# xyfJASON/ctrlora

Measured on NVIDIA H100. Metric: ddim_steps_per_sec, higher is better.
Workload: dtype fp16 (fp32 accumulate)

## Files before the change

ctrlora_b200/csrc/gemm_sm90.cu:

```cuda
#include "gemm_sm90.cuh"
#include "wgmma.cuh"
#include "ctrlora_b200.h"
#include <stdio.h>
#include <string.h>

namespace ctrl {

__device__ __forceinline__ uint32_t pack_h2(float a, float b) {
    __half2 h = __floats2half2_rn(a, b);
    return *reinterpret_cast<uint32_t*>(&h);
}

template <int CW>
__device__ __forceinline__ void epilogue_chunk(const GemmKParams& p, float* v, int c, int bn_out, int n0, bool row_ok,
                                               long long m, int img, int tok) {
    const int nbase = n0 + c;
    const bool full_chunk = (c + CW <= bn_out) && (nbase + CW <= p.N);
    if (!row_ok) return;
    if (p.rowbias) {
        const float* rb = p.rowbias + static_cast<long long>(img) * p.rowbias_ld + nbase;
        if (full_chunk && (p.rowbias_ld & 3) == 0) {
#pragma unroll
            for (int q = 0; q < CW / 4; ++q) {
                const float4 b4 = __ldg(reinterpret_cast<const float4*>(rb) + q);
                v[4 * q] += b4.x; v[4 * q + 1] += b4.y; v[4 * q + 2] += b4.z; v[4 * q + 3] += b4.w;
            }
        } else {
#pragma unroll
            for (int j = 0; j < CW; ++j)
                if (nbase + j < p.N) v[j] += __ldg(rb + j);
        }
    }
    if (p.out_scale != 1.0f) {
#pragma unroll
        for (int j = 0; j < CW; ++j) v[j] *= p.out_scale;
    }
    if (p.residual && p.residual_f32) {
        const float* rp = reinterpret_cast<const float*>(p.residual) + m * p.ldr + nbase;
        if (full_chunk && (p.ldr & 3) == 0) {
#pragma unroll
            for (int q = 0; q < CW / 4; ++q) {
                const float4 r4 = __ldg(reinterpret_cast<const float4*>(rp) + q);
                v[4 * q] += r4.x; v[4 * q + 1] += r4.y; v[4 * q + 2] += r4.z; v[4 * q + 3] += r4.w;
            }
        } else {
#pragma unroll
            for (int j = 0; j < CW; ++j)
                if (c + j < bn_out && nbase + j < p.N) v[j] += rp[j];
        }
    } else if (p.residual) {
        const __half* rp = p.residual + m * p.ldr + nbase;
        if (full_chunk && (p.ldr & 7) == 0) {
            uint4 u[CW / 8];
#pragma unroll
            for (int q = 0; q < CW / 8; ++q) u[q] = __ldg(reinterpret_cast<const uint4*>(rp) + q);
#pragma unroll
            for (int q = 0; q < CW / 8; ++q) {
                const __half2* h = reinterpret_cast<const __half2*>(&u[q]);
#pragma unroll
                for (int e = 0; e < 4; ++e) {
                    const float2 f = __half22float2(h[e]);
                    v[q * 8 + e * 2] += f.x;
                    v[q * 8 + e * 2 + 1] += f.y;
                }
            }
        } else {
#pragma unroll
            for (int j = 0; j < CW; ++j)
                if (c + j < bn_out && nbase + j < p.N) v[j] += __half2float(rp[j]);
        }
    }
    int seg = 0, nloc = nbase;
    if (p.seg_width > 0) { seg = nbase / p.seg_width; nloc = nbase - seg * p.seg_width; }
    if (p.transposed[seg]) {
        __half* o = reinterpret_cast<__half*>(p.out[seg]) + (static_cast<long long>(img) * p.seg_width + nloc) * p.tok_pad + tok;
#pragma unroll
        for (int j = 0; j < CW; ++j)
            if (c + j < bn_out && nbase + j < p.N) o[static_cast<long long>(j) * p.tok_pad] = __float2half_rn(v[j]);
        if (p.dup_out) {
            __half* o2 = p.dup_out + m * p.dup_ld + nloc;
#pragma unroll
            for (int j = 0; j < CW; ++j)
                if (c + j < bn_out && nbase + j < p.N) o2[j] = __float2half_rn(v[j]);
        }
    } else if (p.out_f32) {
        float* o = reinterpret_cast<float*>(p.out[seg]) + m * p.ldc + nloc;
        if (full_chunk && (p.ldc & 3) == 0) {
#pragma unroll
            for (int q = 0; q < CW / 4; ++q)
                reinterpret_cast<float4*>(o)[q] = make_float4(v[q * 4], v[q * 4 + 1], v[q * 4 + 2], v[q * 4 + 3]);
        } else {
#pragma unroll
            for (int j = 0; j < CW; ++j)
                if (c + j < bn_out && nbase + j < p.N) o[j] = v[j];
        }
    } else {
        __half* o = reinterpret_cast<__half*>(p.out[seg]) + m * p.ldc + nloc;
        if (full_chunk && (p.ldc & 7) == 0) {
#pragma unroll
            for (int q = 0; q < CW / 8; ++q) {
                uint4 u;
                u.x = pack_h2(v[q * 8 + 0], v[q * 8 + 1]);
                u.y = pack_h2(v[q * 8 + 2], v[q * 8 + 3]);
                u.z = pack_h2(v[q * 8 + 4], v[q * 8 + 5]);
                u.w = pack_h2(v[q * 8 + 6], v[q * 8 + 7]);
                reinterpret_cast<uint4*>(o)[q] = u;
            }
        } else {
#pragma unroll
            for (int j = 0; j < CW; ++j)
                if (c + j < bn_out && nbase + j < p.N) o[j] = __float2half_rn(v[j]);
        }
    }
}

struct GemmUnit {
    int mt, nt, it0, it1, ks, slot;
};
__device__ __forceinline__ GemmUnit gemm_unit(const GemmKParams& p, int u, int m_tiles, int k_iters) {
    GemmUnit w;
    int tile;
    if (u < p.tiles_whole) {
        tile = u;
        w.ks = 0; w.slot = -1; w.it0 = 0; w.it1 = k_iters;
    } else {
        const int v = u - p.tiles_whole;
        w.slot = v / p.splits;
        w.ks = v - w.slot * p.splits;
        tile = p.tiles_whole + w.slot;
        w.it0 = w.ks * p.kiters_per_split;
        w.it1 = min(k_iters, w.it0 + p.kiters_per_split);
    }
    w.mt = tile % m_tiles;
    w.nt = tile / m_tiles;
    return w;
}

__device__ __forceinline__ uint32_t epi_addr(uint32_t base, int r, int col) {
    return base + static_cast<uint32_t>(r * (GEMM_EPI_COLS * 4) + ((((col >> 2) ^ (r & 7)) << 4) | ((col & 3) << 2)));
}

template <bool GEGLU, int BN>
__global__ void __launch_bounds__(GEMM_THREADS, 1)
gemm_wgmma_kernel(const __grid_constant__ CUtensorMap tmA, const __grid_constant__ CUtensorMap tmB,
                  const __grid_constant__ CUtensorMap tmA2, const __grid_constant__ CUtensorMap tmB2,
                  const __grid_constant__ GemmKParams p) {
    constexpr int BN_OUT = GEGLU ? BN / 2 : BN;
    constexpr int NACC = BN / 2;
    constexpr int BOX = GEGLU || BN > 256 ? BN / 2 : BN;
    extern __shared__ uint8_t smem_raw[];
    uint8_t* smem = reinterpret_cast<uint8_t*>((reinterpret_cast<uintptr_t>(smem_raw) + 1023) & ~uintptr_t(1023));
    uint64_t* bars = reinterpret_cast<uint64_t*>(smem + GEMM_SMEM_DATA + GEMM_EPI_BYTES);
    uint64_t* full = bars;
    uint64_t* empty = bars + GEMM_MAX_STAGES;
    volatile int* last_flag = reinterpret_cast<volatile int*>(bars + 2 * GEMM_MAX_STAGES);

    pdl_launch_dependents();
    const int warp = uniform_warp_idx();
    const int lane = threadIdx.x & 31;
    const int nstages = p.stages;
    if (threadIdx.x == 0) {
        tma_prefetch_desc(&tmA);
        tma_prefetch_desc(&tmB);
        if (p.kchunks2 > 0) {
            tma_prefetch_desc(&tmA2);
            tma_prefetch_desc(&tmB2);
        }
        for (int i = 0; i < nstages; ++i) {
            mbar_init(&full[i], 1);
            mbar_init(&empty[i], GEMM_CONSUMERS);
        }
        fence_barrier_init();
    }
    __syncthreads();
    pdl_wait();

    const int m_tiles = p.tiles_w * p.tiles_h * p.tiles_b;
    const int main_iters = p.taps * p.kchunks;
    const int k_iters = main_iters + p.kchunks2;

    if (warp < 4) {
        setmaxnreg_dec<GEMM_PRODUCER_REGS>();
        if (warp == 0 && elect_one()) {
            const uint32_t tx_bytes = GEMM_A_BYTES + BN * 128;
            int s = 0;
            uint32_t phase = 0;
            for (int u = blockIdx.x; u < p.units; u += gridDim.x) {
                const GemmUnit w = gemm_unit(p, u, m_tiles, k_iters);
                const int tw = w.mt % p.tiles_w, th = (w.mt / p.tiles_w) % p.tiles_h, tb = w.mt / (p.tiles_w * p.tiles_h);
                const int w0 = tw * p.bw - p.pad, h0 = th * p.bh - p.pad, b0 = tb * p.nb, n0 = w.nt * BN_OUT;
                for (int it = w.it0; it < w.it1; ++it) {
                    mbar_wait_nocall(&empty[s], phase ^ 1);
                    uint8_t* dst = smem + s * p.stage_bytes;
                    mbar_expect_tx(&full[s], tx_bytes);
                    if (it < main_iters) {
                        const int tap = it / p.kchunks, kc = it - tap * p.kchunks, ky = tap / p.kw, kx = tap - ky * p.kw;
                        tma_load_4d(dst, &tmA, &full[s], kc * GEMM_BK, w0 + kx, h0 + ky, b0);
                        tma_load_3d(dst + GEMM_A_BYTES, &tmB, &full[s], kc * GEMM_BK, tap, n0);
                        if (BOX < BN)
                            tma_load_3d(dst + GEMM_A_BYTES + BOX * 128, &tmB, &full[s], kc * GEMM_BK, tap, GEGLU ? p.N + n0 : n0 + BOX);
                    } else {
                        const int c0 = (it - main_iters) * GEMM_BK;
                        tma_load_4d(dst, &tmA2, &full[s], c0, w0 + p.pad, h0 + p.pad, b0);
                        tma_load_3d(dst + GEMM_A_BYTES, &tmB2, &full[s], c0, 0, n0);
                        if (BOX < BN) tma_load_3d(dst + GEMM_A_BYTES + BOX * 128, &tmB2, &full[s], c0, 0, n0 + BOX);
                    }
                    if (++s == nstages) { s = 0; phase ^= 1; }
                }
            }
        }
        return;
    }

    setmaxnreg_inc<GEMM_CONSUMER_REGS>();
    const int ct = threadIdx.x - 128;
    const int wg = ct >> 7, t = ct & 127;
    const uint32_t smem0 = smem_u32(smem);
    const uint32_t stg = smem0 + GEMM_SMEM_DATA + wg * (64 * GEMM_EPI_COLS * 4);
    const int fr = ((t >> 5) << 4) + (lane >> 2), cq = 2 * (lane & 3);
    const int er = t & 63, eh = t >> 6;
    const long long slice = static_cast<long long>(GEMM_BM) * BN;
    int s = 0;
    uint32_t phase = 0;
    for (int u = blockIdx.x; u < p.units; u += gridDim.x) {
        const GemmUnit w = gemm_unit(p, u, m_tiles, k_iters);
        float acc[NACC];
#pragma unroll
        for (int i = 0; i < NACC; ++i) acc[i] = 0.f;
        int prev = -1;
        for (int it = w.it0; it < w.it1; ++it) {
            mbar_wait_nocall(&full[s], phase);
            const uint32_t a_base = smem0 + s * p.stage_bytes + wg * 64 * 128;
            const uint32_t b_base = smem0 + s * p.stage_bytes + GEMM_A_BYTES;
            wgmma_fence();
#pragma unroll
            for (int k = 0; k < GEMM_BK / 16; ++k) {
                const uint32_t sc = (it > w.it0 || k > 0) ? 1u : 0u;
                if constexpr (BN > 256) {
                    WgmmaSS<BN / 2, 0, 0>::mma(acc, wgmma_desc_kmajor(a_base + 32 * k), wgmma_desc_kmajor(b_base + 32 * k), sc);
                    WgmmaSS<BN / 2, 0, 0>::mma(acc + NACC / 2, wgmma_desc_kmajor(a_base + 32 * k),
                                               wgmma_desc_kmajor(b_base + (BN / 2) * 128 + 32 * k), sc);
                } else {
                    WgmmaSS<BN, 0, 0>::mma(acc, wgmma_desc_kmajor(a_base + 32 * k), wgmma_desc_kmajor(b_base + 32 * k), sc);
                }
            }
            wgmma_commit();
            wgmma_wait<1>();
            if (prev >= 0) mbar_arrive(&empty[prev]);
            prev = s;
            if (++s == nstages) { s = 0; phase ^= 1; }
        }
        wgmma_wait<0>();
        wgmma_fence_regs<NACC>(acc);
        mbar_arrive(&empty[prev]);

        if (w.slot >= 0) {
            float* frag0 = p.ws + static_cast<long long>(w.slot) * p.splits * slice + ct * 4;
#pragma unroll
            for (int i = 0; i < NACC / 4; ++i)
                __stcg(reinterpret_cast<float4*>(frag0 + w.ks * slice + i * (GEMM_CONSUMERS * 4)),
                       make_float4(acc[4 * i], acc[4 * i + 1], acc[4 * i + 2], acc[4 * i + 3]));
            __threadfence();
            named_bar_sync(1, GEMM_CONSUMERS);
            if (ct == 0) {
                const unsigned int old = atomicAdd(&p.counters[w.slot], 1u);
                const int last = (old == static_cast<unsigned int>(p.splits - 1));
                if (last) p.counters[w.slot] = 0;
                *last_flag = last;
            }
            named_bar_sync(1, GEMM_CONSUMERS);
            if (!*last_flag) continue;
            __threadfence();
#pragma unroll
            for (int i = 0; i < NACC / 4; ++i) {
                float4 t4 = make_float4(0.f, 0.f, 0.f, 0.f);
                for (int sl = 0; sl < p.splits; ++sl) {
                    const float4 x4 = __ldcg(reinterpret_cast<const float4*>(frag0 + sl * slice + i * (GEMM_CONSUMERS * 4)));
                    t4.x += x4.x; t4.y += x4.y; t4.z += x4.z; t4.w += x4.w;
                }
                acc[4 * i] = t4.x; acc[4 * i + 1] = t4.y; acc[4 * i + 2] = t4.z; acc[4 * i + 3] = t4.w;
            }
        }

        const int n0 = w.nt * BN_OUT;
        auto bias_geglu = [&](int i) {
#pragma unroll
            for (int e = 0; e < 2; ++e) {
                const int n = n0 + 8 * i + cq + e;
                float bv = 0.f, bg = 0.f;
                if (p.bias && n < p.N) {
                    bv = __ldg(p.bias + n);
                    if (GEGLU) bg = __ldg(p.bias + p.N + n);
                }
                acc[4 * i + e] += bv;
                acc[4 * i + 2 + e] += bv;
                if (GEGLU) {
                    acc[4 * i + e] *= gelu_erf_f(acc[4 * (i + BN_OUT / 8) + e] + bg);
                    acc[4 * i + 2 + e] *= gelu_erf_f(acc[4 * (i + BN_OUT / 8) + 2 + e] + bg);
                }
            }
        };
        if (GEGLU) {
#pragma unroll
            for (int i = 0; i < BN_OUT / 8; ++i) bias_geglu(i);
        }
        const int tw = w.mt % p.tiles_w, th = (w.mt / p.tiles_w) % p.tiles_h, tb = w.mt / (p.tiles_w * p.tiles_h);
        const int r = wg * 64 + er;
        const int iw = r % p.bw, ih = (r / p.bw) % p.bh, ib = r / (p.bw * p.bh);
        const int gw = tw * p.bw + iw, gh = th * p.bh + ih, gb = tb * p.nb + ib;
        const bool row_ok = gw < p.W && gh < p.H && gb < p.Bn;
        const long long m = (static_cast<long long>(gb) * p.H + gh) * p.W + gw;
        const int img = row_ok ? static_cast<int>(m / p.rows_per_img) : 0;
        const int tok = row_ok ? static_cast<int>(m % p.rows_per_img) : 0;
        constexpr int NSLAB = (BN_OUT + GEMM_EPI_COLS - 1) / GEMM_EPI_COLS;
#pragma unroll
        for (int sl = 0; sl < NSLAB; ++sl) {
            const int s0 = sl * GEMM_EPI_COLS;
#pragma unroll
            for (int j = 0; j < GEMM_EPI_COLS / 8; ++j) {
                const int i = sl * (GEMM_EPI_COLS / 8) + j;
                if (i >= BN_OUT / 8) break;
                if (!GEGLU) bias_geglu(i);
                const int col = 8 * j + cq;
                asm volatile("st.shared.v2.f32 [%0], {%1, %2};" ::"r"(epi_addr(stg, fr, col)), "f"(acc[4 * i]), "f"(acc[4 * i + 1])
                             : "memory");
                asm volatile("st.shared.v2.f32 [%0], {%1, %2};" ::"r"(epi_addr(stg, fr + 8, col)), "f"(acc[4 * i + 2]),
                             "f"(acc[4 * i + 3])
                             : "memory");
            }
            named_bar_sync(2 + wg, 128);
            constexpr int CW = BN_OUT > 128 ? 16 : 32;
#pragma unroll
            for (int c1 = 0; c1 < 32; c1 += CW) {
                const int c = s0 + 32 * eh + c1;
                if (c < BN_OUT) {
                    float v[CW];
#pragma unroll
                    for (int q = 0; q < CW / 4; ++q) {
                        const float4 x = lds128f(epi_addr(stg, er, 32 * eh + c1 + 4 * q));
                        v[4 * q] = x.x; v[4 * q + 1] = x.y; v[4 * q + 2] = x.z; v[4 * q + 3] = x.w;
                    }
                    epilogue_chunk<CW>(p, v, c, BN_OUT, n0, row_ok, m, img, tok);
                }
            }
            named_bar_sync(2 + wg, 128);
        }
    }
}

typedef CUresult (*PFN_tmapEncodeTiled)(CUtensorMap*, CUtensorMapDataType, cuuint32_t, void*, const cuuint64_t*,
                                        const cuuint64_t*, const cuuint32_t*, const cuuint32_t*, CUtensorMapInterleave,
                                        CUtensorMapSwizzle, CUtensorMapL2promotion, CUtensorMapFloatOOBfill);

PFN_tmapEncodeTiled get_tmap_encoder() {
    static PFN_tmapEncodeTiled fn = nullptr;
    if (!fn) {
        void* ptr = nullptr;
        cudaDriverEntryPointQueryResult q;
        if (cudaGetDriverEntryPoint("cuTensorMapEncodeTiled", &ptr, cudaEnableDefault, &q) != cudaSuccess ||
            q != cudaDriverEntryPointSuccess)
            return nullptr;
        fn = reinterpret_cast<PFN_tmapEncodeTiled>(ptr);
    }
    return fn;
}

static int make_tmap_f16_sw(CUtensorMap* map, const void* base, int rank, const uint64_t* dims, const uint64_t* strides_bytes,
                            const uint32_t* box, CUtensorMapSwizzle swz);
int make_tmap_f16(CUtensorMap* map, const void* base, int rank, const uint64_t* dims, const uint64_t* strides_bytes,
                  const uint32_t* box) {
    return make_tmap_f16_sw(map, base, rank, dims, strides_bytes, box, CU_TENSOR_MAP_SWIZZLE_128B);
}
static int make_tmap_f16_sw(CUtensorMap* map, const void* base, int rank, const uint64_t* dims, const uint64_t* strides_bytes,
                            const uint32_t* box, CUtensorMapSwizzle swz) {
    PFN_tmapEncodeTiled enc = get_tmap_encoder();
    if (!enc) return CTRLORA_ERR_TMAP;
    cuuint64_t gdim[5], gstr[4];
    cuuint32_t bx[5], es[5];
    for (int i = 0; i < rank; ++i) { gdim[i] = dims[i]; bx[i] = box[i]; es[i] = 1; }
    for (int i = 0; i + 1 < rank; ++i) gstr[i] = strides_bytes[i];
    CUresult r = enc(map, CU_TENSOR_MAP_DATA_TYPE_FLOAT16, rank, const_cast<void*>(base), gdim, gstr, bx, es,
                     CU_TENSOR_MAP_INTERLEAVE_NONE, swz, CU_TENSOR_MAP_L2_PROMOTION_L2_256B,
                     CU_TENSOR_MAP_FLOAT_OOB_FILL_NONE);
    if (r != CUDA_SUCCESS) {
        fprintf(stderr, "ctrlora: cuTensorMapEncodeTiled failed (%d) rank %d dims", (int)r, rank);
        for (int i = 0; i < rank; ++i) fprintf(stderr, " %llu", (unsigned long long)dims[i]);
        fprintf(stderr, " box");
        for (int i = 0; i < rank; ++i) fprintf(stderr, " %u", box[i]);
        fprintf(stderr, "\n");
        return CTRLORA_ERR_TMAP;
    }
    return CTRLORA_OK;
}

static int pow2_floor(int x) {
    int p = 1;
    while (p * 2 <= x) p *= 2;
    return p;
}

static int g_num_sms = 0;
static int g_sm_limit = 0;

int persistent_sms() {
    if (g_num_sms == 0) {
        int dev = 0;
        cudaGetDevice(&dev);
        cudaDeviceGetAttribute(&g_num_sms, cudaDevAttrMultiProcessorCount, dev);
        if (g_num_sms <= 0) return 0;
    }
    return g_sm_limit > 0 && g_sm_limit < g_num_sms ? g_sm_limit : g_num_sms;
}

constexpr double GEMM_L2_BPC = 40.0;
constexpr double GEMM_EPI_FIXED = 600.0;
constexpr double GEMM_EPI_PER_COL = 12.0;
constexpr double GEMM_SPLIT_PER_COL = 12.0;
constexpr int GEMM_MAX_AUTO_SPLIT = 8;
static constexpr int GEMM_WIDE_MIN_KITERS = 40;
static bool g_attr_set = false;

template <bool GEGLU, int BN>
static cudaError_t launch_gemm(dim3 grid, cudaStream_t stream, const CUtensorMap& tmA, const CUtensorMap& tmB,
                               const CUtensorMap& tmA2, const CUtensorMap& tmB2, const GemmKParams& p) {
    return launch_pdl(gemm_wgmma_kernel<GEGLU, BN>, grid, dim3(GEMM_THREADS), (size_t)GEMM_SMEM_BYTES, stream, tmA, tmB, tmA2,
                      tmB2, p);
}
template <bool GEGLU, int BN>
static bool set_smem_attr() {
    return cudaFuncSetAttribute(gemm_wgmma_kernel<GEGLU, BN>, cudaFuncAttributeMaxDynamicSharedMemorySize, GEMM_SMEM_BYTES) ==
           cudaSuccess;
}

}

using namespace ctrl;

extern "C" int ctrlora_gemm_f16(const ctrlora_gemm_args* a, void* stream_) {
    cudaStream_t stream = reinterpret_cast<cudaStream_t>(stream_);
    if (!a || !a->a || !a->w || !a->out[0]) return CTRLORA_ERR_ARG;
    if (a->a_c % 8 != 0 || a->a_ld % 8 != 0) return CTRLORA_ERR_ARG;
    if (a->kh != a->kw || (a->kh != 1 && a->kh != 3)) return CTRLORA_ERR_UNSUPPORTED;
    if (a->bf16) return CTRLORA_ERR_UNSUPPORTED;
    GemmKParams p;
    memset(&p, 0, sizeof(p));
    p.W = a->a_w; p.H = a->a_h; p.Bn = a->a_b;
    p.bw = pow2_floor(p.W < 128 ? p.W : 128);
    p.bh = pow2_floor(p.H < 128 / p.bw ? p.H : 128 / p.bw);
    p.nb = 128 / (p.bw * p.bh);
    p.tiles_w = (p.W + p.bw - 1) / p.bw;
    p.tiles_h = (p.H + p.bh - 1) / p.bh;
    p.tiles_b = (p.Bn + p.nb - 1) / p.nb;
    p.N = a->n;
    p.taps = a->kh * a->kw; p.kw = a->kw; p.pad = a->pad;
    p.kchunks = (a->a_c + GEMM_BK - 1) / GEMM_BK;
    p.kchunks2 = a->a2 ? (a->a2_c + GEMM_BK - 1) / GEMM_BK : 0;
    p.geglu = a->geglu;
    const int sms = persistent_sms();
    if (sms <= 0) return CTRLORA_ERR_CUDA;
    const int m_tiles = p.tiles_w * p.tiles_h * p.tiles_b;
    const int k_iters = p.taps * p.kchunks + p.kchunks2;
    const bool explicit_split = a->split_k > 0;
    auto plan = [&](int cand, int S, int* s_eff, int* whole) -> double {
        const int bnt = p.geglu ? 2 * cand : cand;
        const long long tiles = (long long)m_tiles * ((p.N + cand - 1) / cand);
        const int kps = (k_iters + S - 1) / S;
        *s_eff = (k_iters + kps - 1) / kps;
        long long w = *s_eff == 1 ? tiles : explicit_split ? 0 : (tiles / sms) * sms;
        const long long tail = tiles - w;
        if (*s_eff > 1 && (!a->splitk_ws || !a->splitk_counters || tail == 0 ||
                           tail * *s_eff * GEMM_BM * bnt * 4 > a->splitk_ws_bytes || tail > a->splitk_counters_len))
            return -1.0;
        *whole = (int)w;
        const double step = fmax(4.0 * bnt, (double)(GEMM_A_BYTES + bnt * 128) / GEMM_L2_BPC);
        const double epi = GEMM_EPI_FIXED + GEMM_EPI_PER_COL * cand;
        const double t_whole = k_iters * step + epi;
        const double t_split = kps * step + epi + GEMM_SPLIT_PER_COL * bnt * (1 + *s_eff);
        return (double)((w + sms - 1) / sms) * t_whole + (double)((tail * *s_eff + sms - 1) / sms) * t_split;
    };
    int bn_out = 0, splits = 1, tiles_whole = 0;
    double best_cost = -1;
    static const int kWidths[] = {GEMM_MAX_BN, 256, 128, 64, 32};
    for (int wi = 0; wi < 5; ++wi) {
        const int cand = p.geglu ? kWidths[wi] / 2 : kWidths[wi];
        if (cand < 32) continue;
        if (a->block_n > 0 && cand != a->block_n) continue;
        if (a->block_n <= 0 && kWidths[wi] > 256 && k_iters < GEMM_WIDE_MIN_KITERS) continue;
        if (a->seg_width > 0 && a->seg_width % cand != 0) continue;
        for (int S = explicit_split ? a->split_k : 1; S <= (explicit_split ? a->split_k : GEMM_MAX_AUTO_SPLIT); ++S) {
            int s_eff, whole;
            const double cost = plan(cand, S, &s_eff, &whole);
            if (cost < 0) continue;
            if (best_cost < 0 || cost < best_cost) { best_cost = cost; bn_out = cand; splits = s_eff; tiles_whole = whole; }
        }
    }
    if (bn_out <= 0) {
        return CTRLORA_ERR_ARG;
    }
    p.BN = p.geglu ? 2 * bn_out : bn_out;
    p.n_tiles = (p.N + bn_out - 1) / bn_out;
    p.kiters_per_split = (k_iters + splits - 1) / splits;
    p.splits = (k_iters + p.kiters_per_split - 1) / p.kiters_per_split;
    p.tiles_whole = tiles_whole;
    p.units = tiles_whole + (m_tiles * p.n_tiles - tiles_whole) * p.splits;
    if (p.splits > 1) {
        p.ws = a->splitk_ws;
        p.counters = a->splitk_counters;
    }
    p.stage_bytes = GEMM_A_BYTES + ((p.BN * 128 + 1023) / 1024) * 1024;
    p.stages = GEMM_SMEM_DATA / p.stage_bytes;
    if (p.stages > GEMM_MAX_STAGES) p.stages = GEMM_MAX_STAGES;
    for (int i = 0; i < 3; ++i) { p.out[i] = a->out[i]; p.transposed[i] = a->transposed[i]; }
    p.seg_width = a->seg_width;
    p.ldc = a->ldc; p.out_f32 = a->out_f32;
    p.bias = a->bias; p.rowbias = a->rowbias;
    p.rows_per_img = a->rows_per_img > 0 ? a->rows_per_img : p.W * p.H;
    p.residual = reinterpret_cast<const __half*>(a->residual); p.ldr = a->ldr;
    p.residual_f32 = a->residual_f32;
    p.rowbias_ld = a->rowbias_ld > 0 ? a->rowbias_ld : a->n;
    p.out_scale = a->out_scale;
    p.head_dim = a->head_dim; p.tok_pad = a->tok_pad;
    p.dup_out = reinterpret_cast<__half*>(a->dup_out); p.dup_ld = a->dup_ld;

    const int b_box = p.geglu || p.BN > 256 ? p.BN / 2 : p.BN;
    CUtensorMap tmA, tmB, tmA2, tmB2;
    {
        uint64_t dims[4] = {(uint64_t)a->a_c, (uint64_t)p.W, (uint64_t)p.H, (uint64_t)p.Bn};
        uint64_t str[3] = {(uint64_t)a->a_ld * 2, (uint64_t)a->a_ld * 2 * p.W, (uint64_t)a->a_ld * 2 * p.W * p.H};
        uint32_t box[4] = {GEMM_BK, (uint32_t)p.bw, (uint32_t)p.bh, (uint32_t)p.nb};
        int rc = make_tmap_f16(&tmA, a->a, 4, dims, str, box);
        if (rc) return rc;
        const uint64_t rows = p.geglu ? 2ull * p.N : (uint64_t)p.N;
        uint64_t wd[3] = {(uint64_t)a->a_c, (uint64_t)p.taps, rows};
        uint64_t ws[2] = {(uint64_t)a->a_c * 2, (uint64_t)a->a_c * 2 * p.taps};
        uint32_t wb[3] = {GEMM_BK, 1, (uint32_t)b_box};
        rc = make_tmap_f16(&tmB, a->w, 3, wd, ws, wb);
        if (rc) return rc;
    }
    if (a->a2) {
        if (!a->w2 || a->a2_c % 8 != 0 || a->a2_ld % 8 != 0 || p.geglu) return CTRLORA_ERR_ARG;
        uint64_t dims[4] = {(uint64_t)a->a2_c, (uint64_t)p.W, (uint64_t)p.H, (uint64_t)p.Bn};
        uint64_t str[3] = {(uint64_t)a->a2_ld * 2, (uint64_t)a->a2_ld * 2 * p.W, (uint64_t)a->a2_ld * 2 * p.W * p.H};
        uint32_t box[4] = {GEMM_BK, (uint32_t)p.bw, (uint32_t)p.bh, (uint32_t)p.nb};
        int rc = make_tmap_f16(&tmA2, a->a2, 4, dims, str, box);
        if (rc) return rc;
        uint64_t wd[3] = {(uint64_t)a->a2_c, 1, (uint64_t)p.N};
        uint64_t ws[2] = {(uint64_t)a->a2_c * 2, (uint64_t)a->a2_c * 2};
        uint32_t wb[3] = {GEMM_BK, 1, (uint32_t)b_box};
        rc = make_tmap_f16(&tmB2, a->w2, 3, wd, ws, wb);
        if (rc) return rc;
    } else {
        tmA2 = tmA;
        tmB2 = tmB;
    }
    if (!g_attr_set) {
        if (!set_smem_attr<false, 32>() || !set_smem_attr<false, 64>() || !set_smem_attr<false, 128>() ||
            !set_smem_attr<false, 256>() || !set_smem_attr<false, 320>() || !set_smem_attr<true, 64>() ||
            !set_smem_attr<true, 128>() || !set_smem_attr<true, 256>() || !set_smem_attr<true, 320>())
            return CTRLORA_ERR_CUDA;
        g_attr_set = true;
    }
    const dim3 grid((unsigned)(p.units < sms ? p.units : sms));
    cudaError_t lrc;
    if (p.geglu) lrc = p.BN == 64  ? launch_gemm<true, 64>(grid, stream, tmA, tmB, tmA2, tmB2, p)
                     : p.BN == 128 ? launch_gemm<true, 128>(grid, stream, tmA, tmB, tmA2, tmB2, p)
                     : p.BN == 256 ? launch_gemm<true, 256>(grid, stream, tmA, tmB, tmA2, tmB2, p)
                                   : launch_gemm<true, 320>(grid, stream, tmA, tmB, tmA2, tmB2, p);
    else lrc = p.BN == 32  ? launch_gemm<false, 32>(grid, stream, tmA, tmB, tmA2, tmB2, p)
             : p.BN == 64  ? launch_gemm<false, 64>(grid, stream, tmA, tmB, tmA2, tmB2, p)
             : p.BN == 128 ? launch_gemm<false, 128>(grid, stream, tmA, tmB, tmA2, tmB2, p)
             : p.BN == 256 ? launch_gemm<false, 256>(grid, stream, tmA, tmB, tmA2, tmB2, p)
                           : launch_gemm<false, 320>(grid, stream, tmA, tmB, tmA2, tmB2, p);
    if (lrc != cudaSuccess) return CTRLORA_ERR_CUDA;
    return cudaGetLastError() == cudaSuccess ? CTRLORA_OK : CTRLORA_ERR_CUDA;
}

extern "C" int ctrlora_set_sm_limit(int limit) {
    if (limit < 0) return CTRLORA_ERR_ARG;
    g_sm_limit = limit;
    return CTRLORA_OK;
}
```

ctrlora_b200/csrc/gemm_sm90.cuh:

```cuda
#pragma once
#include "common.cuh"

namespace ctrl {

constexpr int GEMM_BM = 128;
constexpr int GEMM_BK = 64;
constexpr int GEMM_MAX_BN = 320;
constexpr int GEMM_MAX_STAGES = 8;
constexpr int GEMM_A_BYTES = GEMM_BM * GEMM_BK * 2;
constexpr int GEMM_THREADS = 384;
constexpr int GEMM_CONSUMERS = 256;
constexpr int GEMM_PRODUCER_REGS = 40;
constexpr int GEMM_CONSUMER_REGS = 232;
constexpr int GEMM_SMEM_DATA = 192 * 1024;
constexpr int GEMM_EPI_COLS = 64;
constexpr int GEMM_EPI_BYTES = 2 * 64 * GEMM_EPI_COLS * 4;
constexpr int GEMM_SMEM_BYTES = GEMM_SMEM_DATA + GEMM_EPI_BYTES + 1024  + 256 ;

struct GemmKParams {
    int W, H, Bn;
    int bw, bh, nb;
    int tiles_w, tiles_h, tiles_b;
    int N;
    int BN;
    int n_tiles;
    int taps, kw, pad;
    int kchunks;
    int kchunks2;
    int geglu;
    int stages, stage_bytes;
    int units, tiles_whole;
    int splits, kiters_per_split;
    float* ws;
    unsigned int* counters;
    void* out[3];
    int seg_width;
    int transposed[3];
    int ldc;
    int out_f32;
    const float* bias;
    const float* rowbias;
    int rows_per_img;
    int rowbias_ld;
    int residual_f32;
    const __half* residual;
    int ldr;
    float out_scale;
    int head_dim, tok_pad;
    __half* dup_out;
    int dup_ld;
};

}
```

Measured before the change: 31.37.

## Add TMA-based epilogue with residual prefetch and slot ring overlapping stores

Adds a dedicated producer warp that TMA-loads residual slabs into a ring of shared-memory epilogue slots and TMA-stores the finished fp16 output slabs, so consumers write swizzled results to smem instead of doing scattered global stores. Shared memory is repartitioned between mainloop stages and epilogue slots, and a new BN=160 tile width is added for short-K GEMMs. Alignment checks in the fallback epilogue now test pointer alignment directly. This aims to overlap epilogue global traffic with the next tile's mainloop, at the cost of fewer pipeline stages and extra barrier complexity.

```diff
diff --git a/ctrlora_b200/csrc/gemm_sm90.cu b/ctrlora_b200/csrc/gemm_sm90.cu
--- a/ctrlora_b200/csrc/gemm_sm90.cu
+++ b/ctrlora_b200/csrc/gemm_sm90.cu
@@ -6,6 +6,7 @@
 
 namespace ctrl {
 
+__device__ __forceinline__ bool aligned16(const void* ptr) { return (reinterpret_cast<uintptr_t>(ptr) & 15) == 0; }
 __device__ __forceinline__ uint32_t pack_h2(float a, float b) {
     __half2 h = __floats2half2_rn(a, b);
     return *reinterpret_cast<uint32_t*>(&h);
@@ -19,7 +20,7 @@
     if (!row_ok) return;
     if (p.rowbias) {
         const float* rb = p.rowbias + static_cast<long long>(img) * p.rowbias_ld + nbase;
-        if (full_chunk && (p.rowbias_ld & 3) == 0) {
+        if (full_chunk && aligned16(rb)) {
 #pragma unroll
             for (int q = 0; q < CW / 4; ++q) {
                 const float4 b4 = __ldg(reinterpret_cast<const float4*>(rb) + q);
@@ -37,7 +38,7 @@
     }
     if (p.residual && p.residual_f32) {
         const float* rp = reinterpret_cast<const float*>(p.residual) + m * p.ldr + nbase;
-        if (full_chunk && (p.ldr & 3) == 0) {
+        if (full_chunk && aligned16(rp)) {
 #pragma unroll
             for (int q = 0; q < CW / 4; ++q) {
                 const float4 r4 = __ldg(reinterpret_cast<const float4*>(rp) + q);
@@ -50,7 +51,7 @@
         }
     } else if (p.residual) {
         const __half* rp = p.residual + m * p.ldr + nbase;
-        if (full_chunk && (p.ldr & 7) == 0) {
+        if (full_chunk && aligned16(rp)) {
             uint4 u[CW / 8];
 #pragma unroll
             for (int q = 0; q < CW / 8; ++q) u[q] = __ldg(reinterpret_cast<const uint4*>(rp) + q);
@@ -85,7 +86,7 @@
         }
     } else if (p.out_f32) {
         float* o = reinterpret_cast<float*>(p.out[seg]) + m * p.ldc + nloc;
-        if (full_chunk && (p.ldc & 3) == 0) {
+        if (full_chunk && aligned16(o)) {
 #pragma unroll
             for (int q = 0; q < CW / 4; ++q)
                 reinterpret_cast<float4*>(o)[q] = make_float4(v[q * 4], v[q * 4 + 1], v[q * 4 + 2], v[q * 4 + 3]);
@@ -96,7 +97,7 @@
         }
     } else {
         __half* o = reinterpret_cast<__half*>(p.out[seg]) + m * p.ldc + nloc;
-        if (full_chunk && (p.ldc & 7) == 0) {
+        if (full_chunk && aligned16(o)) {
 #pragma unroll
             for (int q = 0; q < CW / 8; ++q) {
                 uint4 u;
@@ -140,20 +141,40 @@
     return base + static_cast<uint32_t>(r * (GEMM_EPI_COLS * 4) + ((((col >> 2) ^ (r & 7)) << 4) | ((col & 3) << 2)));
 }
 
+__host__ __device__ constexpr int gemm_slab_cols(int bn_out) { return bn_out % 64 == 0 ? 64 : 32; }
+__device__ __forceinline__ uint32_t lds32(uint32_t addr) {
+    uint32_t v;
+    asm volatile("ld.shared.b32 %0, [%1];" : "=r"(v) : "r"(addr) : "memory");
+    return v;
+}
+__device__ __forceinline__ void sts32(uint32_t addr, uint32_t v) {
+    asm volatile("st.shared.b32 [%0], %1;" ::"r"(addr), "r"(v) : "memory");
+}
+__device__ __forceinline__ float2 h2_to_f2(uint32_t u) { return __half22float2(*reinterpret_cast<const __half2*>(&u)); }
+
 template <bool GEGLU, int BN>
 __global__ void __launch_bounds__(GEMM_THREADS, 1)
 gemm_wgmma_kernel(const __grid_constant__ CUtensorMap tmA, const __grid_constant__ CUtensorMap tmB,
                   const __grid_constant__ CUtensorMap tmA2, const __grid_constant__ CUtensorMap tmB2,
+                  const __grid_constant__ CUtensorMap tmR, const __grid_constant__ CUtensorMap tmO0,
+                  const __grid_constant__ CUtensorMap tmO1, const __grid_constant__ CUtensorMap tmO2,
                   const __grid_constant__ GemmKParams p) {
     constexpr int BN_OUT = GEGLU ? BN / 2 : BN;
     constexpr int NACC = BN / 2;
     constexpr int BOX = GEGLU || BN > 256 ? BN / 2 : BN;
+    constexpr int SW = gemm_slab_cols(BN_OUT);
+    constexpr int NSLAB_TMA = BN_OUT / SW;
+    constexpr int SLOT = GEMM_BM * SW * 2;
     extern __shared__ uint8_t smem_raw[];
     uint8_t* smem = reinterpret_cast<uint8_t*>((reinterpret_cast<uintptr_t>(smem_raw) + 1023) & ~uintptr_t(1023));
-    uint64_t* bars = reinterpret_cast<uint64_t*>(smem + GEMM_SMEM_DATA + GEMM_EPI_BYTES);
+    uint8_t* ring = smem + p.epi_slots * SLOT;
+    uint64_t* bars = reinterpret_cast<uint64_t*>(smem + GEMM_SMEM_DATA);
     uint64_t* full = bars;
     uint64_t* empty = bars + GEMM_MAX_STAGES;
-    volatile int* last_flag = reinterpret_cast<volatile int*>(bars + 2 * GEMM_MAX_STAGES);
+    uint64_t* slot_ready = bars + 2 * GEMM_MAX_STAGES;
+    uint64_t* slot_done = slot_ready + GEMM_MAX_SLOTS;
+    uint64_t* drained = slot_done + GEMM_MAX_SLOTS;
+    volatile int* last_flag = reinterpret_cast<volatile int*>(drained + 1);
 
     pdl_launch_dependents();
     const int warp = uniform_warp_idx();
@@ -170,6 +191,11 @@
             mbar_init(&full[i], 1);
             mbar_init(&empty[i], GEMM_CONSUMERS);
         }
+        for (int i = 0; i < p.epi_slots; ++i) {
+            mbar_init(&slot_ready[i], 1);
+            mbar_init(&slot_done[i], GEMM_CONSUMERS);
+        }
+        mbar_init(drained, 1);
         fence_barrier_init();
     }
     __syncthreads();
@@ -191,7 +217,7 @@
                 const int w0 = tw * p.bw - p.pad, h0 = th * p.bh - p.pad, b0 = tb * p.nb, n0 = w.nt * BN_OUT;
                 for (int it = w.it0; it < w.it1; ++it) {
                     mbar_wait_nocall(&empty[s], phase ^ 1);
-                    uint8_t* dst = smem + s * p.stage_bytes;
+                    uint8_t* dst = ring + s * p.stage_bytes;
                     mbar_expect_tx(&full[s], tx_bytes);
                     if (it < main_iters) {
                         const int tap = it / p.kchunks, kc = it - tap * p.kchunks, ky = tap / p.kw, kx = tap - ky * p.kw;
@@ -208,6 +234,46 @@
                     if (++s == nstages) { s = 0; phase ^= 1; }
                 }
             }
+        } else if (warp == 1 && p.tma_tiles > 0 && elect_one()) {
+            const int nslots = p.epi_slots;
+            auto open = [&](int u, int j, int slot) {
+                if (!p.residual) { mbar_arrive(&slot_ready[slot]); return; }
+                const int mt = u % m_tiles, nt = u / m_tiles;
+                const int tw = mt % p.tiles_w, th = (mt / p.tiles_w) % p.tiles_h, tb = mt / (p.tiles_w * p.tiles_h);
+                mbar_expect_tx(&slot_ready[slot], GEMM_BM * SW * 2);
+                tma_load_4d(smem + slot * SLOT, &tmR, &slot_ready[slot], nt * BN_OUT + j * SW, tw * p.bw, th * p.bh,
+                            tb * p.nb);
+            };
+            int ou = blockIdx.x, oj = 0;
+            for (int k = 0; k < nslots && ou < p.tma_tiles; ++k) {
+                open(ou, oj, k);
+                if (++oj == NSLAB_TMA) { oj = 0; ou += gridDim.x; }
+            }
+            int slot = 0, prev_slot = -1;
+            uint32_t phase = 0;
+            for (int u = blockIdx.x; u < p.tma_tiles; u += gridDim.x) {
+                const int mt = u % m_tiles, nt = u / m_tiles;
+                const int tw = mt % p.tiles_w, th = (mt / p.tiles_w) % p.tiles_h, tb = mt / (p.tiles_w * p.tiles_h);
+                for (int j = 0; j < NSLAB_TMA; ++j) {
+                    int col = nt * BN_OUT + j * SW, seg = 0;
+                    if (p.seg_width > 0) { seg = col / p.seg_width; col -= seg * p.seg_width; }
+                    mbar_wait_nocall(&slot_done[slot], phase);
+                    tma_store_4d(seg == 0 ? &tmO0 : seg == 1 ? &tmO1 : &tmO2, smem_u32(smem + slot * SLOT), col,
+                                 tw * p.bw, th * p.bh, tb * p.nb);
+                    bulk_commit_group();
+                    if (prev_slot >= 0) {
+                        bulk_wait_group_read<1>();
+                        if (ou < p.tma_tiles) {
+                            open(ou, oj, prev_slot);
+                            if (++oj == NSLAB_TMA) { oj = 0; ou += gridDim.x; }
+                        }
+                    }
+                    prev_slot = slot;
+                    if (++slot == nslots) { slot = 0; phase ^= 1; }
+                }
+            }
+            bulk_wait_group<0>();
+            mbar_arrive(drained);
         }
         return;
     }
@@ -215,13 +281,12 @@
     setmaxnreg_inc<GEMM_CONSUMER_REGS>();
     const int ct = threadIdx.x - 128;
     const int wg = ct >> 7, t = ct & 127;
-    const uint32_t smem0 = smem_u32(smem);
-    const uint32_t stg = smem0 + GEMM_SMEM_DATA + wg * (64 * GEMM_EPI_COLS * 4);
+    const uint32_t ring0 = smem_u32(ring);
     const int fr = ((t >> 5) << 4) + (lane >> 2), cq = 2 * (lane & 3);
     const int er = t & 63, eh = t >> 6;
     const long long slice = static_cast<long long>(GEMM_BM) * BN;
     int s = 0;
-    uint32_t phase = 0;
+    uint32_t phase = 0, slot_pos = 0;
     for (int u = blockIdx.x; u < p.units; u += gridDim.x) {
         const GemmUnit w = gemm_unit(p, u, m_tiles, k_iters);
         float acc[NACC];
@@ -230,8 +295,8 @@
         int prev = -1;
         for (int it = w.it0; it < w.it1; ++it) {
             mbar_wait_nocall(&full[s], phase);
-            const uint32_t a_base = smem0 + s * p.stage_bytes + wg * 64 * 128;
-            const uint32_t b_base = smem0 + s * p.stage_bytes + GEMM_A_BYTES;
+            const uint32_t a_base = ring0 + s * p.stage_bytes + wg * 64 * 128;
+            const uint32_t b_base = ring0 + s * p.stage_bytes + GEMM_A_BYTES;
             wgmma_fence();
 #pragma unroll
             for (int k = 0; k < GEMM_BK / 16; ++k) {
@@ -305,6 +370,57 @@
             for (int i = 0; i < BN_OUT / 8; ++i) bias_geglu(i);
         }
         const int tw = w.mt % p.tiles_w, th = (w.mt / p.tiles_w) % p.tiles_h, tb = w.mt / (p.tiles_w * p.tiles_h);
+        if (u < p.tma_tiles) {
+            const uint32_t row_off = (wg * 64 + fr) * (SW * 2) + cq * 2, row_x = SW == 64 ? (fr & 7) : ((fr >> 1) & 3);
+            const float* rb0 = nullptr;
+            const float* rb1 = nullptr;
+            if (p.rowbias) {
+                auto row_img = [&](int r) {
+                    const int iw = r % p.bw, ih = (r / p.bw) % p.bh, ib = r / (p.bw * p.bh);
+                    const int gw = tw * p.bw + iw, gh = th * p.bh + ih, gb = tb * p.nb + ib;
+                    if (gw >= p.W || gh >= p.H || gb >= p.Bn) return 0LL;
+                    return ((static_cast<long long>(gb) * p.H + gh) * p.W + gw) / p.rows_per_img;
+                };
+                rb0 = p.rowbias + row_img(wg * 64 + fr) * p.rowbias_ld;
+                rb1 = p.rowbias + row_img(wg * 64 + fr + 8) * p.rowbias_ld;
+            }
+#pragma unroll
+            for (int j = 0; j < NSLAB_TMA; ++j) {
+                const int slot = slot_pos & 0xffff;
+                mbar_wait_nocall(&slot_ready[slot], slot_pos >> 16);
+                const uint32_t sb = ring0 - (p.epi_slots - slot) * SLOT + row_off;
+#pragma unroll
+                for (int c = 0; c < SW / 8; ++c) {
+                    const int i = j * (SW / 8) + c;
+                    if (!GEGLU) bias_geglu(i);
+                    float v00 = acc[4 * i], v01 = acc[4 * i + 1], v10 = acc[4 * i + 2], v11 = acc[4 * i + 3];
+                    const int n = n0 + 8 * i + cq;
+                    if (rb0) {
+                        if (n < p.N) { v00 = __fadd_rn(v00, __ldg(rb0 + n)); v10 = __fadd_rn(v10, __ldg(rb1 + n)); }
+                        if (n + 1 < p.N) { v01 = __fadd_rn(v01, __ldg(rb0 + n + 1)); v11 = __fadd_rn(v11, __ldg(rb1 + n + 1)); }
+                    }
+                    if (p.out_scale != 1.0f) {
+                        v00 = __fmul_rn(v00, p.out_scale); v01 = __fmul_rn(v01, p.out_scale);
+                        v10 = __fmul_rn(v10, p.out_scale); v11 = __fmul_rn(v11, p.out_scale);
+                    }
+                    const uint32_t a0 = sb + ((static_cast<uint32_t>(c) ^ row_x) << 4);
+                    const uint32_t a1 = a0 + 8 * SW * 2;
+                    if (p.residual) {
+                        const float2 r0 = h2_to_f2(lds32(a0)), r1 = h2_to_f2(lds32(a1));
+                        v00 = __fadd_rn(v00, r0.x); v01 = __fadd_rn(v01, r0.y);
+                        v10 = __fadd_rn(v10, r1.x); v11 = __fadd_rn(v11, r1.y);
+                    }
+                    sts32(a0, pack_h2(v00, v01));
+                    sts32(a1, pack_h2(v10, v11));
+                }
+                fence_proxy_async_smem();
+                mbar_arrive(&slot_done[slot]);
+                slot_pos = slot + 1 == p.epi_slots ? (slot_pos & 0x10000) ^ 0x10000 : slot_pos + 1;
+            }
+            continue;
+        }
+        if (p.tma_tiles > 0) mbar_wait_nocall(drained, 0);
+        const uint32_t stg = ring0 - p.epi_slots * SLOT + wg * (64 * GEMM_EPI_COLS * 4);
         const int r = wg * 64 + er;
         const int iw = r % p.bw, ih = (r / p.bw) % p.bh, ib = r / (p.bw * p.bh);
         const int gw = tw * p.bw + iw, gh = th * p.bh + ih, gb = tb * p.nb + ib;
@@ -421,10 +537,9 @@
 static bool g_attr_set = false;
 
 template <bool GEGLU, int BN>
-static cudaError_t launch_gemm(dim3 grid, cudaStream_t stream, const CUtensorMap& tmA, const CUtensorMap& tmB,
-                               const CUtensorMap& tmA2, const CUtensorMap& tmB2, const GemmKParams& p) {
-    return launch_pdl(gemm_wgmma_kernel<GEGLU, BN>, grid, dim3(GEMM_THREADS), (size_t)GEMM_SMEM_BYTES, stream, tmA, tmB, tmA2,
-                      tmB2, p);
+static cudaError_t launch_gemm(dim3 grid, cudaStream_t stream, const CUtensorMap* tm, const GemmKParams& p) {
+    return launch_pdl(gemm_wgmma_kernel<GEGLU, BN>, grid, dim3(GEMM_THREADS), (size_t)GEMM_SMEM_BYTES, stream, tm[0], tm[1],
+                      tm[2], tm[3], tm[4], tm[5], tm[6], tm[7], p);
 }
 template <bool GEGLU, int BN>
 static bool set_smem_attr() {
@@ -480,12 +595,13 @@
     };
     int bn_out = 0, splits = 1, tiles_whole = 0;
     double best_cost = -1;
-    static const int kWidths[] = {GEMM_MAX_BN, 256, 128, 64, 32};
-    for (int wi = 0; wi < 5; ++wi) {
+    static const int kWidths[] = {GEMM_MAX_BN, 256, 160, 128, 64, 32};
+    for (int wi = 0; wi < 6; ++wi) {
         const int cand = p.geglu ? kWidths[wi] / 2 : kWidths[wi];
-        if (cand < 32) continue;
+        if (cand < 32 || (p.geglu && kWidths[wi] == 160)) continue;
         if (a->block_n > 0 && cand != a->block_n) continue;
         if (a->block_n <= 0 && kWidths[wi] > 256 && k_iters < GEMM_WIDE_MIN_KITERS) continue;
+        if (a->block_n <= 0 && kWidths[wi] == 160 && k_iters >= GEMM_WIDE_MIN_KITERS) continue;
         if (a->seg_width > 0 && a->seg_width % cand != 0) continue;
         for (int S = explicit_split ? a->split_k : 1; S <= (explicit_split ? a->split_k : GEMM_MAX_AUTO_SPLIT); ++S) {
             int s_eff, whole;
@@ -507,10 +623,30 @@
         p.ws = a->splitk_ws;
         p.counters = a->splitk_counters;
     }
+    for (int i = 0; i < 3; ++i) { p.out[i] = a->out[i]; p.transposed[i] = a->transposed[i]; }
+    const int n_segs = a->seg_width > 0 ? (p.N + a->seg_width - 1) / a->seg_width : 1;
+    if (n_segs > 3) return CTRLORA_ERR_ARG;
+    auto tma_ok = [](const void* ptr, long long ld) { return (reinterpret_cast<uintptr_t>(ptr) & 15) == 0 && ld % 8 == 0; };
+    int tma_segs = 0;
+    while (tma_segs < n_segs && !a->transposed[tma_segs]) ++tma_segs;
+    bool tma_epi = !a->out_f32 && tma_segs > 0 && (!a->residual || (!a->residual_f32 && tma_ok(a->residual, a->ldr)));
+    for (int i = 0; i < n_segs; ++i) {
+        if (i < tma_segs ? !a->out[i] || !tma_ok(a->out[i], a->ldc) : !a->transposed[i]) tma_epi = false;
+    }
+    if (tma_epi) {
+        const long long t = tma_segs == n_segs ? (long long)m_tiles * p.n_tiles : (long long)m_tiles * tma_segs * (a->seg_width / bn_out);
+        p.tma_tiles = (int)(t < tiles_whole ? t : tiles_whole);
+    }
+    const int slab_cols = gemm_slab_cols(bn_out);
+    const int slot_bytes = GEMM_BM * slab_cols * 2;
+    int epi_want = p.tma_tiles > 0 ? (bn_out / slab_cols) * slot_bytes : GEMM_EPI_BYTES;
+    if (epi_want < GEMM_EPI_BYTES) epi_want = GEMM_EPI_BYTES;
     p.stage_bytes = GEMM_A_BYTES + ((p.BN * 128 + 1023) / 1024) * 1024;
-    p.stages = GEMM_SMEM_DATA / p.stage_bytes;
+    p.stages = (GEMM_SMEM_DATA - epi_want) / p.stage_bytes;
+    if (p.stages < 3) p.stages = 3;
     if (p.stages > GEMM_MAX_STAGES) p.stages = GEMM_MAX_STAGES;
-    for (int i = 0; i < 3; ++i) { p.out[i] = a->out[i]; p.transposed[i] = a->transposed[i]; }
+    p.epi_slots = (GEMM_SMEM_DATA - p.stages * p.stage_bytes) / slot_bytes;
+    if (p.epi_slots > GEMM_MAX_SLOTS) p.epi_slots = GEMM_MAX_SLOTS;
     p.seg_width = a->seg_width;
     p.ldc = a->ldc; p.out_f32 = a->out_f32;
     p.bias = a->bias; p.rowbias = a->rowbias;
@@ -523,7 +659,8 @@
     p.dup_out = reinterpret_cast<__half*>(a->dup_out); p.dup_ld = a->dup_ld;
 
     const int b_box = p.geglu || p.BN > 256 ? p.BN / 2 : p.BN;
-    CUtensorMap tmA, tmB, tmA2, tmB2;
+    CUtensorMap tm[8];
+    CUtensorMap &tmA = tm[0], &tmB = tm[1], &tmA2 = tm[2], &tmB2 = tm[3];
     {
         uint64_t dims[4] = {(uint64_t)a->a_c, (uint64_t)p.W, (uint64_t)p.H, (uint64_t)p.Bn};
         uint64_t str[3] = {(uint64_t)a->a_ld * 2, (uint64_t)a->a_ld * 2 * p.W, (uint64_t)a->a_ld * 2 * p.W * p.H};
@@ -553,24 +690,44 @@
         tmA2 = tmA;
         tmB2 = tmB;
     }
+    for (int i = 4; i < 8; ++i) tm[i] = tmA;
+    if (p.tma_tiles > 0) {
+        const CUtensorMapSwizzle swz = slab_cols == 64 ? CU_TENSOR_MAP_SWIZZLE_128B : CU_TENSOR_MAP_SWIZZLE_64B;
+        const uint32_t box[4] = {(uint32_t)slab_cols, (uint32_t)p.bw, (uint32_t)p.bh, (uint32_t)p.nb};
+        auto pixel_map = [&](CUtensorMap* m, const void* base, int cols, long long ld) {
+            uint64_t dims[4] = {(uint64_t)cols, (uint64_t)p.W, (uint64_t)p.H, (uint64_t)p.Bn};
+            uint64_t str[3] = {(uint64_t)ld * 2, (uint64_t)ld * 2 * p.W, (uint64_t)ld * 2 * p.W * p.H};
+            return make_tmap_f16_sw(m, base, 4, dims, str, box, swz);
+        };
+        if (a->residual) {
+            int rc = pixel_map(&tm[4], a->residual, p.N, a->ldr);
+            if (rc) return rc;
+        }
+        for (int i = 0; i < tma_segs; ++i) {
+            const int cols = a->seg_width > 0 ? (p.N - i * a->seg_width < a->seg_width ? p.N - i * a->seg_width : a->seg_width) : p.N;
+            int rc = pixel_map(&tm[5 + i], a->out[i], cols, a->ldc);
+            if (rc) return rc;
+        }
+    }
     if (!g_attr_set) {
         if (!set_smem_attr<false, 32>() || !set_smem_attr<false, 64>() || !set_smem_attr<false, 128>() ||
-            !set_smem_attr<false, 256>() || !set_smem_attr<false, 320>() || !set_smem_attr<true, 64>() ||
+            !set_smem_attr<false, 160>() || !set_smem_attr<false, 256>() || !set_smem_attr<false, 320>() || !set_smem_attr<true, 64>() ||
             !set_smem_attr<true, 128>() || !set_smem_attr<true, 256>() || !set_smem_attr<true, 320>())
             return CTRLORA_ERR_CUDA;
         g_attr_set = true;
     }
     const dim3 grid((unsigned)(p.units < sms ? p.units : sms));
     cudaError_t lrc;
-    if (p.geglu) lrc = p.BN == 64  ? launch_gemm<true, 64>(grid, stream, tmA, tmB, tmA2, tmB2, p)
-                     : p.BN == 128 ? launch_gemm<true, 128>(grid, stream, tmA, tmB, tmA2, tmB2, p)
-                     : p.BN == 256 ? launch_gemm<true, 256>(grid, stream, tmA, tmB, tmA2, tmB2, p)
-                                   : launch_gemm<true, 320>(grid, stream, tmA, tmB, tmA2, tmB2, p);
-    else lrc = p.BN == 32  ? launch_gemm<false, 32>(grid, stream, tmA, tmB, tmA2, tmB2, p)
-             : p.BN == 64  ? launch_gemm<false, 64>(grid, stream, tmA, tmB, tmA2, tmB2, p)
-             : p.BN == 128 ? launch_gemm<false, 128>(grid, stream, tmA, tmB, tmA2, tmB2, p)
-             : p.BN == 256 ? launch_gemm<false, 256>(grid, stream, tmA, tmB, tmA2, tmB2, p)
-                           : launch_gemm<false, 320>(grid, stream, tmA, tmB, tmA2, tmB2, p);
+    if (p.geglu) lrc = p.BN == 64  ? launch_gemm<true, 64>(grid, stream, tm, p)
+                     : p.BN == 128 ? launch_gemm<true, 128>(grid, stream, tm, p)
+                     : p.BN == 256 ? launch_gemm<true, 256>(grid, stream, tm, p)
+                                   : launch_gemm<true, 320>(grid, stream, tm, p);
+    else lrc = p.BN == 32  ? launch_gemm<false, 32>(grid, stream, tm, p)
+             : p.BN == 64  ? launch_gemm<false, 64>(grid, stream, tm, p)
+             : p.BN == 128 ? launch_gemm<false, 128>(grid, stream, tm, p)
+             : p.BN == 160 ? launch_gemm<false, 160>(grid, stream, tm, p)
+             : p.BN == 256 ? launch_gemm<false, 256>(grid, stream, tm, p)
+                           : launch_gemm<false, 320>(grid, stream, tm, p);
     if (lrc != cudaSuccess) return CTRLORA_ERR_CUDA;
     return cudaGetLastError() == cudaSuccess ? CTRLORA_OK : CTRLORA_ERR_CUDA;
 }
diff --git a/ctrlora_b200/csrc/gemm_sm90.cuh b/ctrlora_b200/csrc/gemm_sm90.cuh
--- a/ctrlora_b200/csrc/gemm_sm90.cuh
+++ b/ctrlora_b200/csrc/gemm_sm90.cuh
@@ -12,10 +12,11 @@
 constexpr int GEMM_CONSUMERS = 256;
 constexpr int GEMM_PRODUCER_REGS = 40;
 constexpr int GEMM_CONSUMER_REGS = 232;
-constexpr int GEMM_SMEM_DATA = 192 * 1024;
+constexpr int GEMM_SMEM_DATA = 225 * 1024;
 constexpr int GEMM_EPI_COLS = 64;
 constexpr int GEMM_EPI_BYTES = 2 * 64 * GEMM_EPI_COLS * 4;
-constexpr int GEMM_SMEM_BYTES = GEMM_SMEM_DATA + GEMM_EPI_BYTES + 1024  + 256 ;
+constexpr int GEMM_MAX_SLOTS = 8;
+constexpr int GEMM_SMEM_BYTES = GEMM_SMEM_DATA + 1024  + 512 ;
 
 struct GemmKParams {
     int W, H, Bn;
@@ -29,6 +30,8 @@
     int kchunks2;
     int geglu;
     int stages, stage_bytes;
+    int epi_slots;
+    int tma_tiles;
     int units, tiles_whole;
     int splits, kiters_per_split;
     float* ws;
```

New measurement: 34.63 (median of 6 runs). +10.4%, better.
